# Tencent/yadcc

Measured on NVIDIA B200. Metric: task_assignment_decisions_per_sec, higher is better.
Workload: dtype u32

## Files before the change

yadcc_b200/csrc/fused.cuh:

```cuda
#pragma once
#include "parallel.cuh"
#include <cstddef>
#include "tasks.cuh"

namespace yd {

struct FusedScalars {
  DynParams dyn;
  unsigned long long seq;
  const void* zc_in;
  void* zc_out;
};

struct FusedHostIO {
  unsigned long long done_seq;
  unsigned long long granted;
  uint32_t meta[8];
};

struct FusedArgs {
  FusedScalars sc;
  const FusedScalars* sc_dev;
  FusedHostIO* hio;
  DynParams* dyn_out;
  unsigned long long* clean_keys;
  uint4* clean_zero;
  uint32_t clean_zero_vec;
  const yd_task_req* reqs;
  yd_task_req* reqs_w;
  const uint4* reqs16;
  uint4* reqs16_w;
  TopoView t;
  ClassTable ct;
  ServantArrays sv;
  SlotDecode dec;
  const unsigned long long* m_ptr;
  uint32_t* comp_mode;
  uint32_t n_comps;
  uint32_t n_rtiles, n_ltiles;
  uint32_t* rcls;
  uint32_t* rrank;
  uint32_t* rself;
  uint32_t* rank_cnt;
  uint32_t* list_cnt;
  uint32_t* list_bal;
  uint2* list;
  uint32_t list_cap;
  uint2* rq;
  uint32_t* res;
  RqLayout L;
  uint32_t* bar;
  uint32_t solo, packed_out;
  unsigned long long* look;
  const uint32_t* comp_sv;
  TaskRing ring;
  void* out;
  Counters* counters;
  uint32_t n_servants;
  uint32_t loff_cache_words;
  uint32_t lite;
  unsigned long long* prof;
};

__device__ __forceinline__ unsigned long long fused_now() {
  unsigned long long t;
  asm volatile("mov.u64 %0, %%globaltimer;" : "=l"(t));
  return t;
}
__device__ __forceinline__ void fused_stamp(const FusedArgs& a, int k) {
  if (a.prof && blockIdx.x == 0 && threadIdx.x == 0) a.prof[k] = fused_now();
}

__device__ __forceinline__ void fused_prefetch(const void* p, size_t bytes) {
  const char* base = static_cast<const char*>(p);
  for (size_t off = (size_t(blockIdx.x) * 1024 + threadIdx.x) * 128; off < bytes; off += size_t(gridDim.x) * 1024 * 128) {
    asm volatile("prefetch.global.L2 [%0];" ::"l"(base + off));
  }
}

__device__ __forceinline__ uint32_t fused_atom_add_acq_rel(uint32_t* p, uint32_t v) {
  uint32_t old;
  asm volatile("atom.add.acq_rel.gpu.global.u32 %0, [%1], %2;" : "=r"(old) : "l"(p), "r"(v) : "memory");
  return old;
}
__device__ __forceinline__ uint32_t fused_ld_acquire(const uint32_t* p) {
  uint32_t v;
  asm volatile("ld.acquire.gpu.global.u32 %0, [%1];" : "=r"(v) : "l"(p) : "memory");
  return v;
}
__device__ __forceinline__ void fused_st_release(uint32_t* p, uint32_t v) {
  asm volatile("st.release.gpu.global.u32 [%0], %1;" ::"l"(p), "r"(v) : "memory");
}

__device__ __forceinline__ bool fused_arrive(uint32_t* bar, uint32_t epoch) {
  __shared__ uint32_t s_last;
  __syncthreads();
  if (threadIdx.x == 0) s_last = (fused_atom_add_acq_rel(&bar[0], 1u) + 1 == epoch * gridDim.x) ? 1u : 0u;
  __syncthreads();
  return s_last != 0;
}
__device__ __forceinline__ void fused_release(uint32_t* bar, uint32_t epoch) {
  __syncthreads();
  if (threadIdx.x == 0) fused_st_release(&bar[1], epoch);
}
__device__ __forceinline__ void fused_wait(uint32_t* bar, uint32_t epoch) {
  if (threadIdx.x == 0) {
    while (fused_ld_acquire(&bar[1]) < epoch) {}
  }
  __syncthreads();
}
__device__ __forceinline__ void fused_barrier(uint32_t* bar, uint32_t epoch) {
  __syncthreads();
  if (threadIdx.x == 0) {
    fused_atom_add_acq_rel(&bar[0], 1u);
    const uint32_t want = epoch * gridDim.x;
    while (fused_ld_acquire(&bar[0]) < want) {}
  }
  __syncthreads();
}
__device__ __forceinline__ bool fused_done_last(uint32_t* bar) {
  __shared__ uint32_t s_fin;
  __syncthreads();
  if (threadIdx.x == 0) s_fin = (fused_atom_add_acq_rel(&bar[2], 1u) + 1 == gridDim.x) ? 1u : 0u;
  __syncthreads();
  return s_fin != 0;
}

__device__ __forceinline__ void fused_report(const FusedArgs& a, unsigned long long seq, unsigned long long granted) {
  FusedHostIO* h = a.hio;
  const uint32_t k = threadIdx.x;
  if (k < 8) h->meta[k] = a.ct.meta[k];
  else if (k == 8) { h->granted = granted; h->done_seq = seq; }
}

__device__ __forceinline__ void fused_scan_flat(uint32_t* __restrict__ data, uint32_t cells) {
  __shared__ uint32_t warp_sums[32];
  __shared__ uint32_t carry_s;
  const uint32_t tid = threadIdx.x, lane = tid & 31, warp = tid >> 5;
  if (tid == 0) carry_s = 0;
  __syncthreads();
  for (uint32_t base = 0; base < cells; base += 1024 * 8) {
    const uint32_t i0 = base + tid * 8;
    uint32_t v[8];
#pragma unroll
    for (int k = 0; k < 8; ++k) v[k] = (i0 + k < cells) ? data[i0 + k] : 0;
    uint32_t sum = 0;
#pragma unroll
    for (int k = 0; k < 8; ++k) sum += v[k];
    uint32_t x = sum;
#pragma unroll
    for (int d = 1; d < 32; d <<= 1) {
      const uint32_t y = __shfl_up_sync(0xffffffffu, x, d);
      if (lane >= d) x += y;
    }
    if (lane == 31) warp_sums[warp] = x;
    __syncthreads();
    if (warp == 0) {
      uint32_t w = warp_sums[lane];
#pragma unroll
      for (int d = 1; d < 32; d <<= 1) {
        const uint32_t y = __shfl_up_sync(0xffffffffu, w, d);
        if (lane >= d) w += y;
      }
      warp_sums[lane] = w;
    }
    __syncthreads();
    const uint32_t carry = carry_s;
    uint32_t run = carry + (warp ? warp_sums[warp - 1] : 0) + x - sum;
#pragma unroll
    for (int k = 0; k < 8; ++k) {
      if (i0 + k < cells) data[i0 + k] = run;
      run += v[k];
    }
    __syncthreads();
    if (tid == 1023) carry_s = carry + warp_sums[31];
    __syncthreads();
  }
}

__device__ __forceinline__ uint32_t fused_select(uint32_t q, const FusedArgs& a, const uint32_t* __restrict__ loff) {
  const uint32_t c = a.rcls[q];
  if (c == kNone) return kResEnvNotFound;
  if (a.ct.cls_nelig[c] == 0) return kResEnvNotFound;
  const uint32_t rank = a.rank_cnt[c * a.n_rtiles + q / kRankTile] - a.rank_cnt[c * a.n_rtiles] + a.rrank[q];
  const uint32_t* row = loff + c * a.n_ltiles;
  const uint32_t lb = row[0], le = row[a.n_ltiles];
  if (rank >= le - lb) return kResTimeout;
  const uint32_t target = lb + rank;
  uint32_t lo = 0, hi = a.n_ltiles;
  while (hi - lo > 1) {
    const uint32_t mid = (lo + hi) >> 1;
    if (row[mid] <= target) lo = mid; else hi = mid;
  }
  uint32_t j = target - row[lo];
  const uint4* words = reinterpret_cast<const uint4*>(a.list_bal + (size_t(lo) * a.ct.cls_bound + c) * 32);
  uint32_t w = 0, word = 0;
  bool found = false;
#pragma unroll 1
  for (uint32_t v = 0; v < 8 && !found; ++v) {
    const uint4 x = words[v];
    const uint32_t xs[4] = {x.x, x.y, x.z, x.w};
#pragma unroll
    for (int k = 0; k < 4; ++k) {
      if (!found) {
        const uint32_t p = __popc(xs[k]);
        if (j < p) { found = true; w = v * 4 + k; word = xs[k]; }
        else j -= p;
      }
    }
  }
  const uint32_t bit = __fns(word, 0, (int)j + 1);
  return a.dec.rec[lo * kListTile + w * 32 + bit].x;
}

__device__ __forceinline__ uint32_t fused_select_lite(uint32_t q, const FusedArgs& a, const uint32_t* __restrict__ rows,
                                                       const uint32_t* __restrict__ rpre) {
  const uint32_t c = a.rcls[q];
  if (c == kNone) return kResEnvNotFound;
  if (a.ct.cls_nelig[c] == 0) return kResEnvNotFound;
  const uint32_t target = rpre[c] + a.rrank[q];
  const uint32_t* row = rows + c * (a.n_ltiles + 1);
  if (target >= row[a.n_ltiles]) return kResTimeout;
  uint32_t lo = 0, hi = a.n_ltiles;
  while (hi - lo > 1) {
    const uint32_t mid = (lo + hi) >> 1;
    if (row[mid] <= target) lo = mid; else hi = mid;
  }
  uint32_t j = target - row[lo];
  const uint4* words = reinterpret_cast<const uint4*>(a.list_bal + (size_t(lo) * a.ct.cls_bound + c) * 32);
  uint32_t w = 0, word = 0;
  bool found = false;
#pragma unroll 1
  for (uint32_t v = 0; v < 8 && !found; ++v) {
    const uint4 x = words[v];
    const uint32_t xs[4] = {x.x, x.y, x.z, x.w};
#pragma unroll
    for (int k = 0; k < 4; ++k) {
      if (!found) {
        const uint32_t p = __popc(xs[k]);
        if (j < p) { found = true; w = v * 4 + k; word = xs[k]; }
        else j -= p;
      }
    }
  }
  const uint32_t bit = __fns(word, 0, (int)j + 1);
  return a.dec.rec[lo * kListTile + w * 32 + bit].x;
}

__global__ void __launch_bounds__(1024, 1) k_fused_front(FusedArgs a) {
  extern __shared__ uint32_t s_loff[];
  __shared__ unsigned long long s_seen[64];
  __shared__ DynParams s_dyn;
  __shared__ unsigned long long s_seq, s_zc_in, s_zc_out;
  const uint32_t tid = threadIdx.x, G = gridDim.x;
  if (tid == 0) {
    const FusedScalars sc = a.sc_dev ? *a.sc_dev : a.sc;
    s_dyn = sc.dyn;
    s_seq = sc.seq;
    s_zc_in = reinterpret_cast<unsigned long long>(sc.zc_in);
    s_zc_out = reinterpret_cast<unsigned long long>(sc.zc_out);
    if (blockIdx.x == 0 && a.dyn_out) *a.dyn_out = sc.dyn;
  }
  __syncthreads();
  const uint32_t n = s_dyn.n;
  const uint32_t nb_live = (n + 1023) / 1024;
  const uint32_t m = (uint32_t)*a.m_ptr;
  const uint32_t lt_live = min((m + kListTile - 1) / kListTile, a.n_ltiles);
  const ReqView rv{a.reqs, a.reqs16};

  fused_stamp(a, 0);
  if (tid < 64) s_seen[tid] = kClsEmpty;
  __syncthreads();
  {
    const size_t S4 = size_t(a.n_servants) * 4;
    fused_prefetch(a.dec.rec, size_t(m) * 8);
    fused_prefetch(a.sv.run, S4);
    fused_prefetch(a.sv.version, S4);
    fused_prefetch(a.sv.max_tasks, S4);
    fused_prefetch(a.t.sv_comp, S4);
    fused_prefetch(a.t.sv_local, S4);
    fused_prefetch(a.t.comp_sv, S4);
    if (a.t.sv_emask) fused_prefetch(a.t.sv_emask, S4 * 2);
    else { fused_prefetch(a.t.sv_env_off, S4 + 4); }
  }
  const char* zc_in = reinterpret_cast<const char*>(s_zc_in);
  for (uint32_t tile = blockIdx.x; tile < nb_live; tile += G) {
    const uint32_t q = tile * 1024 + tid;
    if (zc_in) {
      if (a.reqs16) {
        if (q < n) a.reqs16_w[q] = reinterpret_cast<const uint4*>(zc_in)[q];
      } else {
        const uint32_t bytes = min(n - tile * 1024, 1024u) * (uint32_t)sizeof(yd_task_req);
        const char* src = zc_in + size_t(tile) * 1024 * sizeof(yd_task_req);
        char* dst = reinterpret_cast<char*>(const_cast<yd_task_req*>(a.reqs)) + size_t(tile) * 1024 * sizeof(yd_task_req);
        for (uint32_t o = tid * 16; o < bytes; o += 1024 * 16) {
          if (o + 16 <= bytes) *reinterpret_cast<uint4*>(dst + o) = *reinterpret_cast<const uint4*>(src + o);
          else *reinterpret_cast<uint2*>(dst + o) = *reinterpret_cast<const uint2*>(src + o);
        }
      }
      __syncthreads();
    }
    if (q < n) {
      uint32_t env, mv, ip;
      if (a.reqs16) {
        const uint4 w = a.reqs16[q];
        env = w.x; mv = w.y; ip = w.z;
        if (a.reqs_w) {
          uint2* dst = reinterpret_cast<uint2*>(a.reqs_w + q);
          const unsigned long long ns = (unsigned long long)(w.w & 0x7fffffffu) * 1000000ull;
          dst[0] = make_uint2(env, mv);
          dst[1] = make_uint2(ip, (w.w >> 31) ? YD_REQ_FLAG_PREFETCH : 0u);
          dst[2] = make_uint2((uint32_t)ns, (uint32_t)(ns >> 32));
        }
      } else {
        rv.head(q, env, mv);
        ip = rv.ip(q);
      }
      cls_insert_one(env, mv, ip, a.t, a.ct, s_seen);
    }
  }

  fused_stamp(a, 1);
  if (fused_arrive(a.bar, 1)) {
    cls_finalize_block(a.t, a.ct, a.n_comps, a.comp_mode, a.solo);
    fused_release(a.bar, 1);
  } else {
    fused_wait(a.bar, 1);
  }
  if (*reinterpret_cast<volatile uint32_t*>(&a.ct.meta[1]) != 0) {
    if (a.solo && blockIdx.x == 0) fused_report(a, s_seq, 0);
    return;
  }
  const uint32_t ncls = min(a.ct.meta[0], a.ct.cls_bound);
  const uint32_t nlists = min(a.ct.meta[3], a.ct.cls_bound);
  fused_stamp(a, 2);

  {
    const uint32_t items = lt_live + a.n_rtiles + ncls;
    for (uint32_t it = blockIdx.x; it < items; it += G) {
      if (it < lt_live) {
        list_count_tile(it, m, a.dec, a.t, a.ct, a.sv, a.n_ltiles, a.list_cnt, a.list_bal);
      } else if (it < lt_live + a.n_rtiles) {
        const uint32_t tile = it - lt_live;
        if (tile < nb_live) {
          rank_count_tile(tile, rv, n, a.t, a.ct, a.comp_mode, a.n_rtiles, a.rcls, a.rrank, a.rself, a.rank_cnt);
        } else if (tid < a.ct.cls_bound) {
          a.rank_cnt[tid * a.n_rtiles + tile] = 0;
        }
      } else {
        cls_elig_class(it - lt_live - a.n_rtiles, a.t, a.ct, a.sv);
      }
    }
  }

  fused_stamp(a, 3);
  const bool lite = a.solo && a.lite && nlists * (a.n_ltiles + 1) <= a.loff_cache_words;
  if (lite) {
    fused_barrier(a.bar, 2);
  } else if (fused_arrive(a.bar, 2)) {
    fused_scan_flat(a.rank_cnt, ncls * a.n_rtiles + 1);
    fused_scan_flat(a.list_cnt, nlists * a.n_ltiles + 1);
    fused_release(a.bar, 2);
  } else {
    fused_wait(a.bar, 2);
  }

  fused_stamp(a, 4);
  if (!a.solo) {
  for (uint32_t tile = blockIdx.x; tile < lt_live; tile += G) {
    list_fill_tile(tile, m, a.dec, a.t, a.ct, a.n_ltiles, a.list_cnt, a.list_bal, a.list, a.list_cap);
  }

  fused_stamp(a, 5);
  if (fused_arrive(a.bar, 3)) fused_release(a.bar, 3);
  else fused_wait(a.bar, 3);
  if (*reinterpret_cast<volatile uint32_t*>(&a.ct.meta[1]) != 0) return;
  }

  fused_stamp(a, 6);
  const long long now_ns = s_dyn.now_ns;
  TaskRing ring = a.ring;
  ring.next = s_dyn.ring_next;
  void* const out = s_zc_out ? reinterpret_cast<void*>(s_zc_out) : a.out;
  if (a.solo && lite) {
    __shared__ uint32_t s_rpre[kMaxClasses];
    const uint32_t lane = tid & 31, warp = tid >> 5, stride = a.n_ltiles + 1;
    for (uint32_t c = warp; c < nlists; c += 32) {
      uint32_t running = 0;
      for (uint32_t t0 = 0; t0 < a.n_ltiles; t0 += 32) {
        const uint32_t t = t0 + lane;
        const uint32_t v = t < a.n_ltiles ? a.list_cnt[c * a.n_ltiles + t] : 0u;
        uint32_t x = v;
#pragma unroll
        for (int d = 1; d < 32; d <<= 1) {
          const uint32_t y = __shfl_up_sync(0xffffffffu, x, d);
          if (lane >= d) x += y;
        }
        if (t < a.n_ltiles) s_loff[c * stride + t] = running + x - v;
        running += __shfl_sync(0xffffffffu, x, 31);
      }
      if (lane == 0) s_loff[c * stride + a.n_ltiles] = running;
    }
    for (uint32_t tile = blockIdx.x; tile < nb_live; tile += G) {
      __syncthreads();
      for (uint32_t c = warp; c < ncls; c += 32) {
        uint32_t sum = 0;
        for (uint32_t t = lane; t < tile; t += 32) sum += a.rank_cnt[c * a.n_rtiles + t];
        sum = __reduce_add_sync(0xffffffffu, sum);
        if (lane == 0) s_rpre[c] = sum;
      }
      __syncthreads();
      const uint32_t q = tile * 1024 + tid;
      const uint32_t r = q < n ? fused_select_lite(q, a, s_loff, s_rpre) : kResEnvNotFound;
      if (a.packed_out) final_tile<true, true, true>(tile, nb_live - 1, r, n, now_ns, rv, a.look, a.comp_sv, ring, out, a.counters, a.sv.run, a.sv.ever);
      else final_tile<false, true, true>(tile, nb_live - 1, r, n, now_ns, rv, a.look, a.comp_sv, ring, out, a.counters, a.sv.run, a.sv.ever);
    }
  } else if (a.solo) {
    const uint32_t cells = nlists * a.n_ltiles + 1;
    const uint32_t* loff = a.list_cnt;
    if (cells <= a.loff_cache_words) {
      for (uint32_t i = tid; i < cells; i += 1024) s_loff[i] = a.list_cnt[i];
      __syncthreads();
      loff = s_loff;
    }
    for (uint32_t tile = blockIdx.x; tile < nb_live; tile += G) {
      const uint32_t q = tile * 1024 + tid;
      const uint32_t r = q < n ? fused_select(q, a, loff) : kResEnvNotFound;
      if (a.packed_out) final_tile<true, true>(tile, nb_live - 1, r, n, now_ns, rv, a.look, a.comp_sv, ring, out, a.counters, a.sv.run, a.sv.ever);
      else final_tile<false, true>(tile, nb_live - 1, r, n, now_ns, rv, a.look, a.comp_sv, ring, out, a.counters, a.sv.run, a.sv.ever);
    }
  } else {
    for (uint32_t tile = blockIdx.x; tile < nb_live; tile += G) {
      const uint32_t q = tile * 1024 + tid;
      uint32_t v;
      if (q < n && rank_assign_one(q, a.n_rtiles, a.t, a.ct, a.rcls, a.rrank, a.rself, a.rank_cnt, a.list_cnt, a.n_ltiles,
                                   a.list, a.comp_mode, a.rq, a.L, v)) {
        a.res[q] = v;
      }
    }
  }
  fused_stamp(a, 7);
  if (a.solo && fused_done_last(a.bar)) {
    fused_report(a, s_seq, a.counters->granted);
    __syncthreads();
    for (uint32_t i = tid; i < kClsTableSize; i += 1024) a.clean_keys[i] = kClsEmpty;
    for (uint32_t i = tid; i < a.clean_zero_vec; i += 1024) a.clean_zero[i] = make_uint4(0u, 0u, 0u, 0u);
    if (a.prof && tid == 0) a.prof[8] = fused_now();
  }
}

__global__ void __launch_bounds__(256) k_unpack_reqs(const uint4* __restrict__ reqs16, const DynParams* __restrict__ dp,
                                                     yd_task_req* __restrict__ reqs) {
  const uint32_t q = blockIdx.x * blockDim.x + threadIdx.x;
  if (q >= dp->n) return;
  const uint4 w = __ldg(reqs16 + q);
  uint2* dst = reinterpret_cast<uint2*>(reqs + q);
  const unsigned long long ns = (unsigned long long)(w.w & 0x7fffffffu) * 1000000ull;
  dst[0] = make_uint2(w.x, w.y);
  dst[1] = make_uint2(w.z, (w.w >> 31) ? YD_REQ_FLAG_PREFETCH : 0u);
  dst[2] = make_uint2((uint32_t)ns, (uint32_t)(ns >> 32));
}

__global__ void __launch_bounds__(256) k_pack_grants(const uint4* __restrict__ grants, const DynParams* __restrict__ dp,
                                                     TaskRing ring, uint2* __restrict__ out) {
  const uint32_t q = blockIdx.x * blockDim.x + threadIdx.x;
  if (q >= dp->n) return;
  const uint4 g = grants[q];
  uint32_t ordinal = 0;
  if (g.w == YD_STATUS_GRANTED) {
    const unsigned long long xid = ((unsigned long long)g.y << 32) | g.x;
    unsigned long long local = 0;
    ring.loc(xid, &local);
    ordinal = (uint32_t)(local - dp->ring_next);
  }
  out[q] = make_uint2(g.z, (g.w << 30) | ordinal);
}

}
```

yadcc_b200/csrc/tasks.cuh:

```cuda
#pragma once
#include "common.cuh"

namespace yd {


__global__ void __launch_bounds__(1024) k_final_count(const uint32_t* __restrict__ res,
                                                      const DynParams* __restrict__ dp,
                                                      uint32_t* __restrict__ block_counts,
                                                      const uint32_t* __restrict__ abort_flag,
                                                      const uint32_t* __restrict__ comp_sv = nullptr,
                                                      uint32_t* __restrict__ claims = nullptr) {
  if (abort_flag && *abort_flag) return;
  uint32_t q = blockIdx.x * 1024 + threadIdx.x;
  const bool granted = (q < dp->n) && (res[q] < kResTimeout);
  if (claims && granted) atomicAdd(&claims[comp_sv[res[q]]], 1u);
  __shared__ uint32_t warp_cnt[32];
  const uint32_t bal = __ballot_sync(0xffffffffu, granted);
  if ((threadIdx.x & 31) == 0) warp_cnt[threadIdx.x >> 5] = __popc(bal);
  __syncthreads();
  if (threadIdx.x < 32) {
    const uint32_t c = __reduce_add_sync(0xffffffffu, warp_cnt[threadIdx.x]);
    if (threadIdx.x == 0) block_counts[blockIdx.x] = c;
  }
}
// ... 8 lines not shown
  const uint32_t tid = threadIdx.x, lane = tid & 31, warp = tid >> 5;
  if (tid == 0) carry_s = 0;
  __syncthreads();
  for (uint32_t base = 0; base < nb; base += 1024) {
    uint32_t i = base + tid;
    uint32_t v = i < nb ? block_counts[i] : 0;
    uint32_t x = v;
#pragma unroll
    for (int d = 1; d < 32; d <<= 1) {
      uint32_t y = __shfl_up_sync(0xffffffffu, x, d);
      if (lane >= d) x += y;
    }
    if (lane == 31) warp_sums[warp] = x;
    __syncthreads();
    if (warp == 0) {
      uint32_t w = warp_sums[lane];
#pragma unroll
      for (int d = 1; d < 32; d <<= 1) {
        uint32_t y = __shfl_up_sync(0xffffffffu, w, d);
        if (lane >= d) w += y;
      }
      warp_sums[lane] = w;
    }
    __syncthreads();
    uint32_t carry = carry_s;
    if (i < nb) block_counts[i] = (id_prefix ? *id_prefix : 0u) + carry + (warp ? warp_sums[warp - 1] : 0) + x - v;
    __syncthreads();
    if (tid == 1023) carry_s = carry + warp_sums[31];
    __syncthreads();
  }
  if (tid == 0) {
    counters->granted = carry_s;
    counters->alive += carry_s;
  }
}

__global__ void __launch_bounds__(1024) k_final_write(const uint32_t* __restrict__ res,
                                                      const yd_task_req* __restrict__ reqs,
                                                      const DynParams* __restrict__ dp,
                                                      const uint32_t* __restrict__ block_off,
                                                      const uint32_t* __restrict__ comp_sv, TaskRing ring,
                                                      yd_grant* __restrict__ out,
                                                      const uint32_t* __restrict__ abort_flag,
                                                      uint32_t* __restrict__ run,
                                                      unsigned long long* __restrict__ ever) {
  if (abort_flag && *abort_flag) return;
  const uint32_t n = dp->n;
  const long long now_ns = dp->now_ns;
  ring.next = dp->ring_next;
  __shared__ uint32_t warp_cnt[32];
  const uint32_t tid = threadIdx.x, lane = tid & 31, warp = tid >> 5;
  const uint32_t q = blockIdx.x * 1024 + tid;
  uint32_t r = q < n ? res[q] : kResEnvNotFound;
  bool granted = r < kResTimeout;
  if (granted) r = comp_sv[r];
  uint32_t bal = __ballot_sync(0xffffffffu, granted);
  if (lane == 0) warp_cnt[warp] = __popc(bal);
  __syncthreads();
  uint32_t before = 0;
  for (uint32_t w = 0; w < warp; ++w) before += warp_cnt[w];
  before += __popc(bal & ((1u << lane) - 1));
  if (q >= n) return;
  uint4 g;
  if (granted) {
    uint64_t id = ring.next + block_off[blockIdx.x] + before;
    const unsigned long long xid = ring.ext(id);
    g = make_uint4((uint32_t)xid, (uint32_t)(xid >> 32), r, YD_STATUS_GRANTED);
    uint64_t slot = id & ring.mask;
    const yd_task_req rq = reqs[q];
    ring.exp[slot] = now_ns + rq.expires_in_ns;
    ring.srv[slot] = r;
    ring.flags[slot] = kTaskAlive | ((rq.flags & YD_REQ_FLAG_PREFETCH) ? kTaskPrefetch : 0u);
    if (run) {
      atomicAdd(&run[r], 1u);
      atomicAdd(&ever[r], 1ull);
    }
  } else {
    g = make_uint4(0u, 0u, YD_NO_SERVANT,
                   (r == kResTimeout) ? YD_STATUS_TIMEOUT : YD_STATUS_ENVIRONMENT_NOT_FOUND);
  }
  *reinterpret_cast<uint4*>(out + q) = g;
}

template <bool kPacked, bool kPos = false, bool kFlat = false>
__device__ __forceinline__ void final_tile(uint32_t vb, uint32_t last_vb, uint32_t r, uint32_t n, long long now_ns,
                                           const ReqView& reqs, unsigned long long* __restrict__ look,
                                           const uint32_t* __restrict__ comp_sv, const TaskRing& ring,
                                           void* __restrict__ out, Counters* __restrict__ counters,
                                           uint32_t* __restrict__ run, unsigned long long* __restrict__ ever) {
  __shared__ uint32_t warp_cnt[32];
  __shared__ unsigned long long s_excl;
  const uint32_t tid = threadIdx.x, lane = tid & 31, warp = tid >> 5;
  const uint32_t q = vb * 1024 + tid;
  const bool granted = r < kResTimeout;
  if (granted && !kPos) r = comp_sv[r];
  const uint32_t bal = __ballot_sync(0xffffffffu, granted);
  if (lane == 0) warp_cnt[warp] = __popc(bal);
  __syncthreads();
  if (warp == 0) {
    const uint32_t mine = __reduce_add_sync(0xffffffffu, warp_cnt[lane]);
    volatile unsigned long long* vl = look;
    if (lane == 0) { __threadfence(); vl[vb] = (1ull << 62) | mine; }
    unsigned long long excl = 0;
    int at = kFlat ? -1 : (int)vb - 1;
    if (kFlat) {
      for (uint32_t base = 0; base < vb; base += 128) {
        unsigned long long v[4];
        bool missing;
        do {
          missing = false;
#pragma unroll
          for (int k = 0; k < 4; ++k) {
            const uint32_t idx = base + k * 32 + lane;
            v[k] = idx < vb ? vl[idx] : (1ull << 62);
            missing |= (v[k] >> 62) == 0;
          }
        } while (__any_sync(0xffffffffu, missing));
#pragma unroll
        for (int k = 0; k < 4; ++k) excl += v[k] & ((1ull << 62) - 1);
      }
#pragma unroll
      for (int d = 16; d; d >>= 1) excl += __shfl_xor_sync(0xffffffffu, excl, d);
    }
    while (at >= 0) {
      const int idx = at - (int)lane;
      unsigned long long v;
      do {
        v = idx >= 0 ? vl[idx] : (2ull << 62);
      } while (__any_sync(0xffffffffu, (v >> 62) == 0));
      const uint32_t incl = __ballot_sync(0xffffffffu, (v >> 62) == 2);
      const unsigned long long val = v & ((1ull << 62) - 1);
      if (incl) {
        const uint32_t first = __ffs(incl) - 1;
        unsigned long long part = lane <= first ? val : 0ull;
#pragma unroll
        for (int d = 16; d; d >>= 1) part += __shfl_xor_sync(0xffffffffu, part, d);
        excl += part;
        break;
      }
      unsigned long long part = val;
#pragma unroll
      for (int d = 16; d; d >>= 1) part += __shfl_xor_sync(0xffffffffu, part, d);
      excl += part;
      at -= 32;
    }
    if (lane == 0) {
      if (!kFlat) {
        __threadfence();
        vl[vb] = (2ull << 62) | (excl + mine);
      }
      s_excl = excl;
      if (vb == last_vb) {
        counters->granted = excl + mine;
        counters->alive += excl + mine;
      }
    }
  }
  __syncthreads();
  if (q < n) {
    uint32_t before = 0;
    for (uint32_t w = 0; w < warp; ++w) before += warp_cnt[w];
    before += __popc(bal & ((1u << lane) - 1));
    const uint64_t ordinal = s_excl + before;
    uint32_t status;
    if (granted) {
      status = YD_STATUS_GRANTED;
      const uint64_t id = ring.next + ordinal;
      const uint64_t slot = id & ring.mask;
      uint32_t rflags;
      long long expires_in_ns;
      reqs.lease(q, rflags, expires_in_ns);
      ring.exp[slot] = now_ns + expires_in_ns;
      ring.srv[slot] = r;
      ring.flags[slot] = kTaskAlive | ((rflags & YD_REQ_FLAG_PREFETCH) ? kTaskPrefetch : 0u);
      atomicAdd(&run[r], 1u);
      atomicAdd(&ever[r], 1ull);
    } else {
      status = (r == kResTimeout) ? YD_STATUS_TIMEOUT : YD_STATUS_ENVIRONMENT_NOT_FOUND;
      r = YD_NO_SERVANT;
    }
    if (kPacked) {
      reinterpret_cast<uint2*>(out)[q] = make_uint2(r, (status << 30) | (granted ? (uint32_t)ordinal : 0u));
    } else {
      const unsigned long long xid = granted ? ring.ext(ring.next + ordinal) : 0ull;
      reinterpret_cast<uint4*>(out)[q] = make_uint4((uint32_t)xid, (uint32_t)(xid >> 32), r, status);
    }
  }
  __syncthreads();
}

__global__ void __launch_bounds__(1024) k_final_fused(const uint32_t* __restrict__ res,
                                                      const yd_task_req* __restrict__ reqs,
                                                      const DynParams* __restrict__ dp,
                                                      unsigned long long* __restrict__ look, uint32_t nb,
                                                      const uint32_t* __restrict__ comp_sv, TaskRing ring,
                                                      yd_grant* __restrict__ out, Counters* __restrict__ counters,
                                                      const uint32_t* __restrict__ abort_flag,
                                                      uint32_t* __restrict__ run, unsigned long long* __restrict__ ever) {
  if (abort_flag && *abort_flag) return;
  __shared__ uint32_t s_vb;
  if (threadIdx.x == 0) s_vb = (uint32_t)atomicAdd(&look[nb], 1ull);
  __syncthreads();
  const uint32_t vb = s_vb;
  const uint32_t n = dp->n;
  ring.next = dp->ring_next;
  const uint32_t q = vb * 1024 + threadIdx.x;
  final_tile<false>(vb, nb - 1, q < n ? res[q] : kResEnvNotFound, n, dp->now_ns, ReqView{reqs, nullptr}, look, comp_sv, ring, out, counters,
                    run, ever);
}

__global__ void k_apply_claims(uint32_t S, const uint32_t* __restrict__ claims, uint32_t* __restrict__ run,
                               unsigned long long* __restrict__ ever, const uint32_t* __restrict__ abort_flag) {
  if (abort_flag && *abort_flag) return;
  const uint32_t s = blockIdx.x * blockDim.x + threadIdx.x;
  if (s >= S || claims[s] == 0) return;
  run[s] += claims[s];
  ever[s] += claims[s];
}

__global__ void k_free(const unsigned long long* __restrict__ ids, uint32_t n, TaskRing ring,
                       uint32_t* __restrict__ run, Counters* __restrict__ counters) {
  uint32_t i = blockIdx.x * blockDim.x + threadIdx.x;
  if (i >= n) return;
  unsigned long long id;
  if (!ring.loc(ids[i], &id) || id < ring.lo || id >= ring.next) return;
  uint64_t slot = id & ring.mask;
  uint32_t old = atomicExch(&ring.flags[slot], 0u);
  if (old & kTaskAlive) {
    atomicSub(&run[ring.srv[slot]], 1u);
    atomicAdd(&counters->alive, ~0ull);
    if (old & kTaskZombie) atomicAdd(&counters->zombies, ~0ull);
  }
}

__global__ void k_keep_alive(const unsigned long long* __restrict__ ids, uint32_t n, long long now_ns,
                             long long new_expires_in_ns, TaskRing ring, uint8_t* __restrict__ ok) {
  uint32_t i = blockIdx.x * blockDim.x + threadIdx.x;
  if (i >= n) return;
  unsigned long long id;
  uint8_t r = 0;
  if (ring.loc(ids[i], &id) && id >= ring.lo && id < ring.next) {
    uint64_t slot = id & ring.mask;
    uint32_t f = ring.flags[slot];
    if ((f & kTaskAlive) && !(f & kTaskZombie)) {
      ring.exp[slot] = now_ns + new_expires_in_ns;
      r = 1;
    }
  }
  ok[i] = r;
}

__global__ void k_tick(TaskRing ring, long long now_ns, const uint32_t* __restrict__ remap,
                       Counters* __restrict__ counters) {
  unsigned long long id = ring.lo + (unsigned long long)blockIdx.x * blockDim.x + threadIdx.x;
  unsigned long long my_min = ~0ull;
  long long d_alive = 0, d_zombie = 0;
  if (id < ring.next) {
    uint64_t slot = id & ring.mask;
    uint32_t f = ring.flags[slot];
    if (f & kTaskAlive) {
      bool gone = false;
      if (remap) {
        uint32_t np = remap[ring.srv[slot]];
        if (np == kNone) {
          ring.flags[slot] = 0;
          gone = true;
          d_alive = -1;
          if (f & kTaskZombie) d_zombie = -1;
        } else {
          ring.srv[slot] = np;
        }
      }
      if (!gone) {
        my_min = id;
        if (!(f & kTaskZombie) && ring.exp[slot] < now_ns) {
          ring.flags[slot] = f | kTaskZombie;
          d_zombie = 1;
        }
      }
    }
  }
  __shared__ unsigned long long s_min[32];
  __shared__ int s_a[32], s_z[32];
  const uint32_t lane = threadIdx.x & 31, warp = threadIdx.x >> 5;
  int a = (int)d_alive, z = (int)d_zombie;
#pragma unroll
  for (int d = 16; d; d >>= 1) {
    unsigned long long o = __shfl_xor_sync(0xffffffffu, my_min, d);
    my_min = o < my_min ? o : my_min;
    a += __shfl_xor_sync(0xffffffffu, a, d);
// ... 106 lines not shown
```

yadcc_b200/csrc/ydsched.cu:

```cuda
#include <algorithm>
#include <chrono>
#include <cstdio>
#include <cstdlib>
#include <cstring>
#include <numeric>
#include <string>
#include <unordered_map>
#include <vector>

#include "common.cuh"
#include "slots.cuh"
#include "radix.cuh"
#include "solve_rowscan.cuh"
#include "solve_stream.cuh"
#include "parallel.cuh"
#include "solve_merge.cuh"
#include "bloom.cuh"
#include "running_index.cuh"
#include "tasks.cuh"
#include "tiny.cuh"
#include "fused.cuh"
#include "filter.cuh"

namespace {
// ... 939 lines not shown
  yd::k_cls_elig<<<ct.cls_bound, 256, 0, st2>>>(t, ct, arr);
  yd::k_rank_count<<<n_rtiles, yd::kRankTile, 0, st2>>>(s->d_reqs.as<yd_task_req>(), dp, t, ct,
                                                         s->d_comp_mode.as<uint32_t>(), n_rtiles,
                                                         s->d_rcls.as<uint32_t>(), s->d_rrank.as<uint32_t>(),
                                                         s->d_rself.as<uint32_t>(), s->d_rank_cnt.as<uint32_t>());
  yd::k_scan_rows<<<ct.cls_bound, 1024, 0, st2>>>(s->d_rank_cnt.as<uint32_t>(), ct.meta, n_rtiles, ScanPub(s, 0));
  YD_CUDA_CHECK(cudaEventRecord(s->ev_join, st2));
  launches += 5;
  if (!s->order_static) {
    launches += LaunchSlotTable(s, true);
    if (s->wide) launches += LaunchSort<unsigned long long>(s, 0, 62);
    else launches += LaunchSort<uint32_t>(s, 3, 30);
  }
  YD_CUDA_CHECK(cudaStreamWaitEvent(st, s->ev_fin, 0));

  const unsigned long long* m_ptr = &s->d_counters.as<Counters>()->slots;
  yd::SlotDecode dec{s->d_sort_v[0].as<uint32_t>(), s->d_slot_owner.as<uint32_t>(), s->d_row_off.as<uint32_t>(),
                     s->d_row_len.as<uint32_t>(), s->d_run.as<uint32_t>(), s->order_static ? 1u : 0u,
                     s->order_static ? s->d_slot_rec.as<uint2>() : nullptr};
  yd::k_list_count<<<n_tiles, yd::kListTile, 0, st>>>(m_ptr, dec, t, ct, arr, n_tiles, list_cnt,
                                                      s->d_list_bal.as<uint32_t>());
  yd::k_scan_rows<<<ct.cls_bound, 1024, 0, st>>>(list_cnt, ct.meta + 3, n_tiles, ScanPub(s, 1));
  yd::k_list_fill<<<n_tiles, yd::kListTile, 0, st>>>(m_ptr, dec, t, ct, n_tiles, list_cnt, s->d_list_bal.as<uint32_t>(),
                                                     s->d_list.as<uint2>(), (uint32_t)(slot_b * 4));
  launches += 3;

  YD_CUDA_CHECK(cudaStreamWaitEvent(st, s->ev_join, 0));
  const yd::RqLayout L = MakeRqLayout(s, 0, N, false);
  yd::k_rank_assign<<<(N + 255) / 256, 256, 0, st>>>(dp, n_rtiles, t, ct, s->d_rcls.as<uint32_t>(),
                                                     s->d_rrank.as<uint32_t>(), s->d_rself.as<uint32_t>(),
                                                     s->d_rank_cnt.as<uint32_t>(), list_cnt,
                                                     n_tiles, s->d_list.as<uint2>(), arr, s->d_comp_mode.as<uint32_t>(),
                                                     s->d_rq.as<uint2>(), s->d_res.as<uint32_t>(), L);
  launches += 1;

  launches += LaunchCoupledSolvers(s, N, slot_b, L);
  return launches;
}

constexpr size_t kFusedLoffCacheWords = 16384;

uint32_t LaunchFused(yd_sched* s, uint32_t N, size_t slot_b, bool capturing, bool solo, bool packed_in, bool packed_out) {
  cudaStream_t st = s->st;
  uint32_t launches = 0;
  const uint32_t n_tiles = (uint32_t)((slot_b + yd::kListTile - 1) / yd::kListTile);
  const uint32_t n_rtiles = (N + yd::kRankTile - 1) / yd::kRankTile;
  yd::FusedArgs a{};
  a.sc = s->fsc;
  a.sc_dev = (capturing && !solo) ? s->d_fsc.as<yd::FusedScalars>() : nullptr;
  if (a.sc_dev) YD_CUDA_CHECK(cudaMemcpyAsync(s->d_fsc.p, s->h_fsc.p, sizeof(yd::FusedScalars), cudaMemcpyHostToDevice, st));
  a.hio = s->report_dev ? s->d_report.as<yd::FusedHostIO>() : s->d_fio;
  a.dyn_out = solo ? nullptr : s->d_dyn.as<yd::DynParams>();
  a.clean_keys = reinterpret_cast<unsigned long long*>(s->d_res.as<uint32_t>() + s->res_words);
  a.clean_zero = reinterpret_cast<uint4*>(static_cast<char*>(s->d_zero.p) + s->z_cls_off);
  a.clean_zero_vec = (uint32_t)((s->z_bytes - s->z_cls_off) / 16);
  a.reqs = s->d_reqs.as<yd_task_req>();
  a.reqs16 = packed_in ? s->d_reqs16.as<uint4>() : nullptr;
  a.reqs16_w = packed_in ? s->d_reqs16.as<uint4>() : nullptr;
  a.reqs_w = (packed_in && !solo) ? s->d_reqs.as<yd_task_req>() : nullptr;
  a.t = MakeTopo(s);
  a.ct = MakeClassTable(s);
  a.sv = s->arrays();
  a.dec = yd::SlotDecode{s->d_sort_v[0].as<uint32_t>(), s->d_slot_owner.as<uint32_t>(), s->d_row_off.as<uint32_t>(),
                         s->d_row_len.as<uint32_t>(), s->d_run.as<uint32_t>(), 1u, s->d_slot_rec.as<uint2>()};
  a.m_ptr = &s->d_counters.as<Counters>()->slots;
  a.comp_mode = s->d_comp_mode.as<uint32_t>();
  a.n_comps = s->n_comps;
  a.n_rtiles = n_rtiles;
  a.n_ltiles = n_tiles;
  a.rcls = s->d_rcls.as<uint32_t>();
  a.rrank = s->d_rrank.as<uint32_t>();
  a.rself = s->d_rself.as<uint32_t>();
  a.rank_cnt = s->d_rank_cnt.as<uint32_t>();
  a.list_cnt = reinterpret_cast<uint32_t*>(static_cast<char*>(s->d_zero.p) + s->z_listcnt_off);
  a.list_bal = s->d_list_bal.as<uint32_t>();
  a.list = s->d_list.as<uint2>();
  a.list_cap = (uint32_t)(slot_b * 4);
  a.rq = s->d_rq.as<uint2>();
  a.res = s->d_res.as<uint32_t>();
  a.L = MakeRqLayout(s, 0, N, false);
  a.bar = reinterpret_cast<uint32_t*>(static_cast<char*>(s->d_zero.p) + s->z_fbar_off);
  a.solo = solo ? 1u : 0u;
  a.packed_out = packed_out ? 1u : 0u;
  a.look = reinterpret_cast<unsigned long long*>(static_cast<char*>(s->d_zero.p) + s->z_final_off);
  a.comp_sv = s->d_comp_sv.as<uint32_t>();
  a.ring = s->ring();
  a.out = packed_out ? s->d_out8.p : s->d_out.p;
  a.counters = s->d_counters.as<Counters>();
  a.n_servants = (uint32_t)s->sv.size();
  a.prof = s->fused_prof ? s->d_fused_prof.as<unsigned long long>() : nullptr;
  YD_CUDA_CHECK(cudaStreamWaitEvent(st, s->ev_h2d, capturing ? cudaEventWaitExternal : 0));
  const uint32_t grid = s->fused_grid;
  const size_t cells = size_t(s->cls_bound) * (n_tiles + 1) + 1;
  const size_t dyn = solo && cells <= kFusedLoffCacheWords ? cells * 4 : 0;
  a.loff_cache_words = (uint32_t)(dyn / 4);
  a.lite = s->fused_lite ? 1u : 0u;
  yd::k_fused_front<<<grid, 1024, dyn, st>>>(a);
  s->last_fused = a;
  s->last_fused_grid = grid;
  s->last_fused_dyn = dyn;
  if (solo && s->report_dev) {
    YD_CUDA_CHECK(cudaMemcpyAsync(s->h_fio, s->d_report.p, sizeof(yd::FusedHostIO), cudaMemcpyDeviceToHost, st));
  }
  launches += 1;
  if (!solo) launches += LaunchCoupledSolvers(s, N, slot_b, a.L);
  return launches;
}

}
}

extern "C++" {
namespace {

uint64_t NextPow2(uint64_t v, uint64_t lo) {
  uint64_t r = lo;
  while (r < v) r <<= 1;
  return r;
}

constexpr uint32_t kFinalFusedMaxBlocks = 2048;

uint32_t FinalPasses(bool solo, uint32_t solver, bool have_work, uint32_t nb) {
  if (solo) return 0;
  return solver == 2 && have_work && nb <= kFinalFusedMaxBlocks ? 1 : 3;
}

uint32_t EnqueueSolve(yd_sched* s, uint32_t Nb, size_t slot_b, uint32_t solver, bool record_events, bool capturing,
                      uint32_t variant = 0, uint32_t packed = 0) {
  cudaStream_t st = s->st;
  const uint32_t S = (uint32_t)s->sv.size();
  const bool have_work = S && s->n_comps;
  const uint32_t nb = (Nb + 1023) / 1024;
  const bool packed_in = packed & 1u, packed_out = packed & 2u;
  uint32_t launches = 0;
  const yd::DynParams* dp = s->d_dyn.as<yd::DynParams>();
  const bool fused = variant && have_work && solver == 2;
  const bool solo = fused && variant >= 2;
  if (!fused) YD_CUDA_CHECK(cudaMemcpyAsync(s->d_dyn.p, s->h_dyn.p, sizeof(yd::DynParams), cudaMemcpyHostToDevice, st));
  if (solo) {
    if (variant == 2) {
      YD_CUDA_CHECK(cudaMemsetAsync(s->d_res.as<uint32_t>() + s->res_words, 0xFF, yd::kClsTableSize * 8, st));
      YD_CUDA_CHECK(cudaMemsetAsync(static_cast<char*>(s->d_zero.p) + s->z_cls_off, 0, s->z_bytes - s->z_cls_off, st));
    }
  } else {
    YD_CUDA_CHECK(cudaMemsetAsync(s->d_res.p, 0xFF, size_t(Nb) * 4 + (solver == 2 ? yd::kClsTableSize * 8 : 0), st));
    if (solver == 2 && have_work) YD_CUDA_CHECK(cudaMemsetAsync(s->d_zero.p, 0, s->z_bytes, st));
  }
  if (record_events) YD_CUDA_CHECK(cudaEventRecord(s->ev[1], st));
  const uint32_t* abort_flag = nullptr;
  if (packed_in && !(variant && have_work && solver == 2)) {
    YD_CUDA_CHECK(cudaStreamWaitEvent(st, s->ev_h2d, capturing ? cudaEventWaitExternal : 0));
    yd::k_unpack_reqs<<<(Nb + 255) / 256, 256, 0, st>>>(s->d_reqs16.as<uint4>(), dp, s->d_reqs.as<yd_task_req>());
    launches += 1;
  }
  if (have_work && solver == 2) {
    if (record_events) YD_CUDA_CHECK(cudaEventRecord(s->ev[2], st));
    if (variant) launches += LaunchFused(s, Nb, slot_b, capturing, variant >= 2, packed_in, packed_out);
    else launches += LaunchStream(s, Nb, slot_b, capturing);
    abort_flag = MakeClassTable(s).meta + 1;
  } else {
    if (have_work) launches += LaunchSlotTable(s, false);
    if (record_events) YD_CUDA_CHECK(cudaEventRecord(s->ev[2], st));
    YD_CUDA_CHECK(cudaStreamWaitEvent(st, s->ev_h2d, capturing ? cudaEventWaitExternal : 0));
    if (have_work) launches += LaunchRowscan(s);
  }
  if (record_events) YD_CUDA_CHECK(cudaEventRecord(s->ev[3], st));
// ... 981 lines not shown
```

Baseline: 2.313 billion.

## Compute per-tile grant offsets from class counts instead of decoupled lookback

In the solo fused path, each tile now derives its exclusive grant offset directly from per-class rank prefix counts, clamped to each class's list length. The grid-wide decoupled lookback chain through the look array is no longer used there, which removes inter-block serialization on the final output pass. The lite and non-lite paths are merged into one loop, the lite list-offset table is staged into shared memory with coalesced loads before the scan, and the bitmap select now loads all eight words unrolled with per-vector popcounts. The cost is an extra per-tile class reduction with block barriers and shared atomics, plus more registers in the select routine.

```diff
diff --git a/yadcc_b200/csrc/fused.cuh b/yadcc_b200/csrc/fused.cuh
--- a/yadcc_b200/csrc/fused.cuh
+++ b/yadcc_b200/csrc/fused.cuh
@@ -51,7 +51,6 @@
   RqLayout L;
   uint32_t* bar;
   uint32_t solo, packed_out;
-  unsigned long long* look;
   const uint32_t* comp_sv;
   TaskRing ring;
   void* out;
@@ -178,73 +177,89 @@
   }
 }
 
-__device__ __forceinline__ uint32_t fused_select(uint32_t q, const FusedArgs& a, const uint32_t* __restrict__ loff) {
-  const uint32_t c = a.rcls[q];
-  if (c == kNone) return kResEnvNotFound;
+__device__ __forceinline__ uint32_t fused_pick(const FusedArgs& a, uint32_t lt, uint32_t c, uint32_t j) {
+  const uint4* words = reinterpret_cast<const uint4*>(a.list_bal + (size_t(lt) * a.ct.cls_bound + c) * 32);
+  uint4 x[8];
+#pragma unroll
+  for (int v = 0; v < 8; ++v) x[v] = words[v];
+  uint32_t p[8];
+#pragma unroll
+  for (int v = 0; v < 8; ++v) p[v] = __popc(x[v].x) + __popc(x[v].y) + __popc(x[v].z) + __popc(x[v].w);
+  uint32_t vsel = 7;
+  bool found = false;
+#pragma unroll
+  for (int v = 0; v < 8; ++v) {
+    if (!found) {
+      if (j < p[v]) { found = true; vsel = v; }
+      else j -= p[v];
+    }
+  }
+  uint4 g = x[0];
+#pragma unroll
+  for (int v = 1; v < 8; ++v) if (vsel == (uint32_t)v) g = x[v];
+  const uint32_t gs[4] = {g.x, g.y, g.z, g.w};
+  uint32_t k = 3, word = g.w;
+  found = false;
+#pragma unroll
+  for (int u = 0; u < 4; ++u) {
+    if (!found) {
+      const uint32_t pc = __popc(gs[u]);
+      if (j < pc) { found = true; k = u; word = gs[u]; }
+      else j -= pc;
+    }
+  }
+  const uint32_t bit = __fns(word, 0, (int)j + 1);
+  return a.dec.rec[lt * kListTile + (vsel * 4 + k) * 32 + bit].x;
+}
+
+__device__ __forceinline__ uint32_t fused_select(const FusedArgs& a, uint32_t c, uint32_t rank, const uint32_t* __restrict__ row) {
   if (a.ct.cls_nelig[c] == 0) return kResEnvNotFound;
-  const uint32_t rank = a.rank_cnt[c * a.n_rtiles + q / kRankTile] - a.rank_cnt[c * a.n_rtiles] + a.rrank[q];
-  const uint32_t* row = loff + c * a.n_ltiles;
-  const uint32_t lb = row[0], le = row[a.n_ltiles];
-  if (rank >= le - lb) return kResTimeout;
+  const uint32_t lb = row[0];
+  if (rank >= row[a.n_ltiles] - lb) return kResTimeout;
   const uint32_t target = lb + rank;
   uint32_t lo = 0, hi = a.n_ltiles;
   while (hi - lo > 1) {
     const uint32_t mid = (lo + hi) >> 1;
     if (row[mid] <= target) lo = mid; else hi = mid;
   }
-  uint32_t j = target - row[lo];
-  const uint4* words = reinterpret_cast<const uint4*>(a.list_bal + (size_t(lo) * a.ct.cls_bound + c) * 32);
-  uint32_t w = 0, word = 0;
-  bool found = false;
-#pragma unroll 1
-  for (uint32_t v = 0; v < 8 && !found; ++v) {
-    const uint4 x = words[v];
-    const uint32_t xs[4] = {x.x, x.y, x.z, x.w};
+  return fused_pick(a, lo, c, target - row[lo]);
+}
+
+__device__ __forceinline__ uint32_t fused_row_sum(const uint32_t* __restrict__ row, uint32_t lim, uint32_t lane) {
+  uint32_t sum = 0;
+  for (uint32_t t0 = 0; t0 < lim; t0 += 128) {
+    uint32_t v[4];
 #pragma unroll
     for (int k = 0; k < 4; ++k) {
-      if (!found) {
-        const uint32_t p = __popc(xs[k]);
-        if (j < p) { found = true; w = v * 4 + k; word = xs[k]; }
-        else j -= p;
-      }
-    }
-  }
-  const uint32_t bit = __fns(word, 0, (int)j + 1);
-  return a.dec.rec[lo * kListTile + w * 32 + bit].x;
-}
-
-__device__ __forceinline__ uint32_t fused_select_lite(uint32_t q, const FusedArgs& a, const uint32_t* __restrict__ rows,
-                                                       const uint32_t* __restrict__ rpre) {
-  const uint32_t c = a.rcls[q];
-  if (c == kNone) return kResEnvNotFound;
-  if (a.ct.cls_nelig[c] == 0) return kResEnvNotFound;
-  const uint32_t target = rpre[c] + a.rrank[q];
-  const uint32_t* row = rows + c * (a.n_ltiles + 1);
-  if (target >= row[a.n_ltiles]) return kResTimeout;
-  uint32_t lo = 0, hi = a.n_ltiles;
-  while (hi - lo > 1) {
-    const uint32_t mid = (lo + hi) >> 1;
-    if (row[mid] <= target) lo = mid; else hi = mid;
-  }
-  uint32_t j = target - row[lo];
-  const uint4* words = reinterpret_cast<const uint4*>(a.list_bal + (size_t(lo) * a.ct.cls_bound + c) * 32);
-  uint32_t w = 0, word = 0;
-  bool found = false;
-#pragma unroll 1
-  for (uint32_t v = 0; v < 8 && !found; ++v) {
-    const uint4 x = words[v];
-    const uint32_t xs[4] = {x.x, x.y, x.z, x.w};
-#pragma unroll
-    for (int k = 0; k < 4; ++k) {
-      if (!found) {
-        const uint32_t p = __popc(xs[k]);
-        if (j < p) { found = true; w = v * 4 + k; word = xs[k]; }
-        else j -= p;
-      }
-    }
-  }
-  const uint32_t bit = __fns(word, 0, (int)j + 1);
-  return a.dec.rec[lo * kListTile + w * 32 + bit].x;
+      const uint32_t t = t0 + k * 32 + lane;
+      v[k] = t < lim ? row[t] : 0u;
+    }
+#pragma unroll
+    for (int k = 0; k < 4; ++k) sum += v[k];
+  }
+  return __reduce_add_sync(0xffffffffu, sum);
+}
+
+__device__ __forceinline__ uint32_t fused_grants_before(const FusedArgs& a, uint32_t tile, uint32_t ncls, bool raw,
+                                                        const uint32_t* __restrict__ loff, uint32_t stride,
+                                                        uint32_t* __restrict__ rpre) {
+  __shared__ uint32_t s_sum;
+  const uint32_t tid = threadIdx.x, lane = tid & 31, warp = tid >> 5;
+  __syncthreads();
+  if (tid == 0) s_sum = 0;
+  __syncthreads();
+  for (uint32_t c = warp; c < ncls; c += 32) {
+    const uint32_t* rc = a.rank_cnt + c * a.n_rtiles;
+    const uint32_t pre = raw ? fused_row_sum(rc, tile, lane) : rc[tile] - rc[0];
+    if (lane == 0) {
+      const uint32_t* row = loff + c * stride;
+      const uint32_t len = a.ct.cls_nelig[c] ? row[a.n_ltiles] - row[0] : 0u;
+      rpre[c] = pre;
+      atomicAdd(&s_sum, min(pre, len));
+    }
+  }
+  __syncthreads();
+  return s_sum;
 }
 
 __global__ void __launch_bounds__(1024, 1) k_fused_front(FusedArgs a) {
@@ -382,52 +397,62 @@
   TaskRing ring = a.ring;
   ring.next = s_dyn.ring_next;
   void* const out = s_zc_out ? reinterpret_cast<void*>(s_zc_out) : a.out;
-  if (a.solo && lite) {
+  if (a.solo) {
     __shared__ uint32_t s_rpre[kMaxClasses];
-    const uint32_t lane = tid & 31, warp = tid >> 5, stride = a.n_ltiles + 1;
-    for (uint32_t c = warp; c < nlists; c += 32) {
-      uint32_t running = 0;
-      for (uint32_t t0 = 0; t0 < a.n_ltiles; t0 += 32) {
-        const uint32_t t = t0 + lane;
-        const uint32_t v = t < a.n_ltiles ? a.list_cnt[c * a.n_ltiles + t] : 0u;
-        uint32_t x = v;
-#pragma unroll
-        for (int d = 1; d < 32; d <<= 1) {
-          const uint32_t y = __shfl_up_sync(0xffffffffu, x, d);
-          if (lane >= d) x += y;
+    const uint32_t lane = tid & 31, warp = tid >> 5;
+    const uint32_t* loff = a.list_cnt;
+    uint32_t stride = a.n_ltiles;
+    if (lite) {
+      const uint32_t nl = a.n_ltiles, cells = nlists * nl;
+      stride = nl + 1;
+      for (uint32_t i0 = tid; i0 < cells; i0 += 4 * 1024) {
+        uint32_t v[4];
+#pragma unroll
+        for (int k = 0; k < 4; ++k) {
+          const uint32_t i = i0 + k * 1024;
+          v[k] = i < cells ? a.list_cnt[i] : 0u;
         }
-        if (t < a.n_ltiles) s_loff[c * stride + t] = running + x - v;
-        running += __shfl_sync(0xffffffffu, x, 31);
-      }
-      if (lane == 0) s_loff[c * stride + a.n_ltiles] = running;
-    }
-    for (uint32_t tile = blockIdx.x; tile < nb_live; tile += G) {
+#pragma unroll
+        for (int k = 0; k < 4; ++k) {
+          const uint32_t i = i0 + k * 1024;
+          if (i < cells) s_loff[i + i / nl] = v[k];
+        }
+      }
       __syncthreads();
-      for (uint32_t c = warp; c < ncls; c += 32) {
-        uint32_t sum = 0;
-        for (uint32_t t = lane; t < tile; t += 32) sum += a.rank_cnt[c * a.n_rtiles + t];
-        sum = __reduce_add_sync(0xffffffffu, sum);
-        if (lane == 0) s_rpre[c] = sum;
-      }
-      __syncthreads();
-      const uint32_t q = tile * 1024 + tid;
-      const uint32_t r = q < n ? fused_select_lite(q, a, s_loff, s_rpre) : kResEnvNotFound;
-      if (a.packed_out) final_tile<true, true, true>(tile, nb_live - 1, r, n, now_ns, rv, a.look, a.comp_sv, ring, out, a.counters, a.sv.run, a.sv.ever);
-      else final_tile<false, true, true>(tile, nb_live - 1, r, n, now_ns, rv, a.look, a.comp_sv, ring, out, a.counters, a.sv.run, a.sv.ever);
-    }
-  } else if (a.solo) {
-    const uint32_t cells = nlists * a.n_ltiles + 1;
-    const uint32_t* loff = a.list_cnt;
-    if (cells <= a.loff_cache_words) {
-      for (uint32_t i = tid; i < cells; i += 1024) s_loff[i] = a.list_cnt[i];
-      __syncthreads();
+      for (uint32_t c = warp; c < nlists; c += 32) {
+        uint32_t* row = s_loff + c * stride;
+        uint32_t running = 0;
+        for (uint32_t t0 = 0; t0 < nl; t0 += 32) {
+          const uint32_t t = t0 + lane;
+          const uint32_t v = t < nl ? row[t] : 0u;
+          uint32_t x = v;
+#pragma unroll
+          for (int d = 1; d < 32; d <<= 1) {
+            const uint32_t y = __shfl_up_sync(0xffffffffu, x, d);
+            if (lane >= d) x += y;
+          }
+          if (t < nl) row[t] = running + x - v;
+          running += __shfl_sync(0xffffffffu, x, 31);
+        }
+        if (lane == 0) row[nl] = running;
+      }
       loff = s_loff;
+    } else {
+      const uint32_t cells = nlists * a.n_ltiles + 1;
+      if (cells <= a.loff_cache_words) {
+        for (uint32_t i = tid; i < cells; i += 1024) s_loff[i] = a.list_cnt[i];
+        loff = s_loff;
+      }
     }
     for (uint32_t tile = blockIdx.x; tile < nb_live; tile += G) {
       const uint32_t q = tile * 1024 + tid;
-      const uint32_t r = q < n ? fused_select(q, a, loff) : kResEnvNotFound;
-      if (a.packed_out) final_tile<true, true>(tile, nb_live - 1, r, n, now_ns, rv, a.look, a.comp_sv, ring, out, a.counters, a.sv.run, a.sv.ever);
-      else final_tile<false, true>(tile, nb_live - 1, r, n, now_ns, rv, a.look, a.comp_sv, ring, out, a.counters, a.sv.run, a.sv.ever);
+      const uint32_t c = q < n ? a.rcls[q] : kNone;
+      const uint32_t rrank = q < n ? a.rrank[q] : 0u;
+      const uint32_t excl = fused_grants_before(a, tile, ncls, lite, loff, stride, s_rpre);
+      const uint32_t r = c != kNone ? fused_select(a, c, s_rpre[c] + rrank, loff + c * stride) : kResEnvNotFound;
+      Counters* const total_to = tile == nb_live - 1 ? a.counters : nullptr;
+      if (a.packed_out) grant_tile<true>(tile, r, n, excl, now_ns, rv, ring, out, a.sv.run, a.sv.ever, total_to);
+      else grant_tile<false>(tile, r, n, excl, now_ns, rv, ring, out, a.sv.run, a.sv.ever, total_to);
     }
   } else {
     for (uint32_t tile = blockIdx.x; tile < nb_live; tile += G) {
diff --git a/yadcc_b200/csrc/tasks.cuh b/yadcc_b200/csrc/tasks.cuh
--- a/yadcc_b200/csrc/tasks.cuh
+++ b/yadcc_b200/csrc/tasks.cuh
@@ -114,7 +114,40 @@
   *reinterpret_cast<uint4*>(out + q) = g;
 }
 
-template <bool kPacked, bool kPos = false, bool kFlat = false>
+template <bool kPacked>
+__device__ __forceinline__ void grant_write(uint32_t q, bool granted, uint32_t r, uint64_t ordinal, long long now_ns,
+                                            uint32_t rflags, long long expires_in_ns, const TaskRing& ring,
+                                            void* __restrict__ out, uint32_t* __restrict__ run,
+                                            unsigned long long* __restrict__ ever) {
+  uint32_t status;
+  if (granted) {
+    status = YD_STATUS_GRANTED;
+    const uint64_t id = ring.next + ordinal;
+    const uint64_t slot = id & ring.mask;
+    ring.exp[slot] = now_ns + expires_in_ns;
+    ring.srv[slot] = r;
+    ring.flags[slot] = kTaskAlive | ((rflags & YD_REQ_FLAG_PREFETCH) ? kTaskPrefetch : 0u);
+    atomicAdd(&run[r], 1u);
+    atomicAdd(&ever[r], 1ull);
+  } else {
+    status = (r == kResTimeout) ? YD_STATUS_TIMEOUT : YD_STATUS_ENVIRONMENT_NOT_FOUND;
+    r = YD_NO_SERVANT;
+  }
+  if (kPacked) {
+    reinterpret_cast<uint2*>(out)[q] = make_uint2(r, (status << 30) | (granted ? (uint32_t)ordinal : 0u));
+  } else {
+    const unsigned long long xid = granted ? ring.ext(ring.next + ordinal) : 0ull;
+    reinterpret_cast<uint4*>(out)[q] = make_uint4((uint32_t)xid, (uint32_t)(xid >> 32), r, status);
+  }
+}
+
+__device__ __forceinline__ uint32_t grant_rank_in_block(const uint32_t* warp_cnt, uint32_t bal) {
+  const uint32_t lane = threadIdx.x & 31, warp = threadIdx.x >> 5;
+  uint32_t before = 0;
+  for (uint32_t w = 0; w < warp; ++w) before += warp_cnt[w];
+  return before + __popc(bal & ((1u << lane) - 1));
+}
+
 __device__ __forceinline__ void final_tile(uint32_t vb, uint32_t last_vb, uint32_t r, uint32_t n, long long now_ns,
                                            const ReqView& reqs, unsigned long long* __restrict__ look,
                                            const uint32_t* __restrict__ comp_sv, const TaskRing& ring,
@@ -125,7 +158,7 @@
   const uint32_t tid = threadIdx.x, lane = tid & 31, warp = tid >> 5;
   const uint32_t q = vb * 1024 + tid;
   const bool granted = r < kResTimeout;
-  if (granted && !kPos) r = comp_sv[r];
+  if (granted) r = comp_sv[r];
   const uint32_t bal = __ballot_sync(0xffffffffu, granted);
   if (lane == 0) warp_cnt[warp] = __popc(bal);
   __syncthreads();
@@ -134,26 +167,7 @@
     volatile unsigned long long* vl = look;
     if (lane == 0) { __threadfence(); vl[vb] = (1ull << 62) | mine; }
     unsigned long long excl = 0;
-    int at = kFlat ? -1 : (int)vb - 1;
-    if (kFlat) {
-      for (uint32_t base = 0; base < vb; base += 128) {
-        unsigned long long v[4];
-        bool missing;
-        do {
-          missing = false;
-#pragma unroll
-          for (int k = 0; k < 4; ++k) {
-            const uint32_t idx = base + k * 32 + lane;
-            v[k] = idx < vb ? vl[idx] : (1ull << 62);
-            missing |= (v[k] >> 62) == 0;
-          }
-        } while (__any_sync(0xffffffffu, missing));
-#pragma unroll
-        for (int k = 0; k < 4; ++k) excl += v[k] & ((1ull << 62) - 1);
-      }
-#pragma unroll
-      for (int d = 16; d; d >>= 1) excl += __shfl_xor_sync(0xffffffffu, excl, d);
-    }
+    int at = (int)vb - 1;
     while (at >= 0) {
       const int idx = at - (int)lane;
       unsigned long long v;
@@ -177,10 +191,8 @@
       at -= 32;
     }
     if (lane == 0) {
-      if (!kFlat) {
-        __threadfence();
-        vl[vb] = (2ull << 62) | (excl + mine);
-      }
+      __threadfence();
+      vl[vb] = (2ull << 62) | (excl + mine);
       s_excl = excl;
       if (vb == last_vb) {
         counters->granted = excl + mine;
@@ -190,33 +202,39 @@
   }
   __syncthreads();
   if (q < n) {
-    uint32_t before = 0;
-    for (uint32_t w = 0; w < warp; ++w) before += warp_cnt[w];
-    before += __popc(bal & ((1u << lane) - 1));
-    const uint64_t ordinal = s_excl + before;
-    uint32_t status;
-    if (granted) {
-      status = YD_STATUS_GRANTED;
-      const uint64_t id = ring.next + ordinal;
-      const uint64_t slot = id & ring.mask;
-      uint32_t rflags;
-      long long expires_in_ns;
-      reqs.lease(q, rflags, expires_in_ns);
-      ring.exp[slot] = now_ns + expires_in_ns;
-      ring.srv[slot] = r;
-      ring.flags[slot] = kTaskAlive | ((rflags & YD_REQ_FLAG_PREFETCH) ? kTaskPrefetch : 0u);
-      atomicAdd(&run[r], 1u);
-      atomicAdd(&ever[r], 1ull);
-    } else {
-      status = (r == kResTimeout) ? YD_STATUS_TIMEOUT : YD_STATUS_ENVIRONMENT_NOT_FOUND;
-      r = YD_NO_SERVANT;
-    }
-    if (kPacked) {
-      reinterpret_cast<uint2*>(out)[q] = make_uint2(r, (status << 30) | (granted ? (uint32_t)ordinal : 0u));
-    } else {
-      const unsigned long long xid = granted ? ring.ext(ring.next + ordinal) : 0ull;
-      reinterpret_cast<uint4*>(out)[q] = make_uint4((uint32_t)xid, (uint32_t)(xid >> 32), r, status);
-    }
+    uint32_t rflags = 0;
+    long long expires_in_ns = 0;
+    if (granted) reqs.lease(q, rflags, expires_in_ns);
+    grant_write<false>(q, granted, r, s_excl + grant_rank_in_block(warp_cnt, bal), now_ns, rflags, expires_in_ns, ring,
+                       out, run, ever);
+  }
+  __syncthreads();
+}
+
+template <bool kPacked>
+__device__ __forceinline__ void grant_tile(uint32_t vb, uint32_t r, uint32_t n, uint32_t excl, long long now_ns,
+                                           const ReqView& reqs, const TaskRing& ring, void* __restrict__ out,
+                                           uint32_t* __restrict__ run, unsigned long long* __restrict__ ever,
+                                           Counters* __restrict__ total_to) {
+  __shared__ uint32_t warp_cnt[32];
+  const uint32_t q = vb * 1024 + threadIdx.x;
+  const bool granted = r < kResTimeout;
+  uint32_t rflags = 0;
+  long long expires_in_ns = 0;
+  if (granted) reqs.lease(q, rflags, expires_in_ns);
+  const uint32_t bal = __ballot_sync(0xffffffffu, granted);
+  if ((threadIdx.x & 31) == 0) warp_cnt[threadIdx.x >> 5] = __popc(bal);
+  __syncthreads();
+  if (total_to && threadIdx.x < 32) {
+    const uint32_t mine = __reduce_add_sync(0xffffffffu, warp_cnt[threadIdx.x]);
+    if (threadIdx.x == 0) {
+      total_to->granted = excl + mine;
+      total_to->alive += excl + mine;
+    }
+  }
+  if (q < n) {
+    grant_write<kPacked>(q, granted, r, (uint64_t)excl + grant_rank_in_block(warp_cnt, bal), now_ns, rflags,
+                         expires_in_ns, ring, out, run, ever);
   }
   __syncthreads();
 }
@@ -237,7 +255,7 @@
   const uint32_t n = dp->n;
   ring.next = dp->ring_next;
   const uint32_t q = vb * 1024 + threadIdx.x;
-  final_tile<false>(vb, nb - 1, q < n ? res[q] : kResEnvNotFound, n, dp->now_ns, ReqView{reqs, nullptr}, look, comp_sv, ring, out, counters,
+  final_tile(vb, nb - 1, q < n ? res[q] : kResEnvNotFound, n, dp->now_ns, ReqView{reqs, nullptr}, look, comp_sv, ring, out, counters,
                     run, ever);
 }
 
diff --git a/yadcc_b200/csrc/ydsched.cu b/yadcc_b200/csrc/ydsched.cu
--- a/yadcc_b200/csrc/ydsched.cu
+++ b/yadcc_b200/csrc/ydsched.cu
@@ -1045,7 +1045,6 @@
   a.bar = reinterpret_cast<uint32_t*>(static_cast<char*>(s->d_zero.p) + s->z_fbar_off);
   a.solo = solo ? 1u : 0u;
   a.packed_out = packed_out ? 1u : 0u;
-  a.look = reinterpret_cast<unsigned long long*>(static_cast<char*>(s->d_zero.p) + s->z_final_off);
   a.comp_sv = s->d_comp_sv.as<uint32_t>();
   a.ring = s->ring();
   a.out = packed_out ? s->d_out8.p : s->d_out.p;
```

New measurement: 2.494 billion (median of 6 runs). 7.8% higher.
